# VachaLab/gorder

Hardware: AMD Instinct MI355X
Metric: trajectory frames/sec (higher is better)
Workload: dtype f32

## Files before the change

### gorder_amd/csrc/gorder_hip.hip

```cpp
#include <hip/hip_runtime.h>

#include <dlfcn.h>

#include <cmath>
#include <cstdio>
#include <cstdlib>
#include <cstring>
#include <mutex>
#include <new>
#include <string>
#include <deque>
#include <vector>

#include "../../include/gorder_hip.h"
#include "gm_math.h"
#include "plan.h"

#pragma clang fp contract(off)

using gorder::DirectItem;
using gorder::Item;
using gorder::kBlock;
using gorder::Plan;
using gorder::Tile;

#include "kernels_common.h"
#include "kernels_bonds.h"
#include "kernels_extras.h"
#include "kernels_leaflets.h"
#include "kernels_normals.h"
#include "kernels_xtc.h"


struct gorder_hip_handle {
    void *traj_cache = nullptr;
    void (*traj_cache_free)(gorder_hip_handle *) = nullptr;
    Plan plan;
    gorder_tables_t tables{};
    int device = 0;
    hipStream_t own_stream = nullptr;
    hipStream_t stream = nullptr;
    Tile *d_tiles = nullptr;
    Item *d_items = nullptr;
    uint32_t *d_tile_slots = nullptr;
    DirectItem *d_direct = nullptr;
    Tile *d_ua_tiles = nullptr;
    gorder::UaItem *d_ua_items = nullptr;
    uint32_t *d_ua_tile_slots = nullptr;
    uint32_t map_nx = 0, map_ny = 0;
    unsigned long long *d_map_sums = nullptr, *d_map_cnts = nullptr;
    unsigned long long *d_map_packed = nullptr;
    unsigned long long *d_map_rec = nullptr;
    size_t map_rec_cap = 0;
    gorder::MapRun *d_ua_runs = nullptr, *d_runs = nullptr;
    uint32_t *d_ua_run_begin = nullptr, *d_run_begin = nullptr;
    Item *d_items_by_slot = nullptr;
    uint32_t *d_ua_item_run = nullptr, *d_item_run = nullptr;
    uint4 *d_lgrid = nullptr;
    LocalRowPre *d_lrowpre = nullptr;
    LocalEdge *d_ledge = nullptr;
    float4 *d_lfinfo = nullptr;
    static constexpr uint32_t kDecidePause = 16;
    uint32_t *d_lsummary = nullptr, *h_lsummary = nullptr;
    hipEvent_t lsummary_written = nullptr;
    bool lsummary_pending = false;
    uint32_t decide_pause = 0;
    uint64_t decide_submits = 0, decide_paused_submits = 0;
    uint32_t *d_lneed = nullptr;
    uint2 *d_ltodo = nullptr;
    size_t map_lds_bytes = 0;
    bool map_staged = false;
    uint64_t map_pending = 0;
    uint64_t map_fold_limit = kMapFoldLimit;
    uint32_t map_max_mol = 1;
    unsigned long long *d_tw_sums = nullptr, *d_tw_cnts = nullptr;
    uint64_t tw_cap = 0;
    ExtraArgs extra{};
    uint32_t *d_geom_group = nullptr;
    float *d_shapes = nullptr;
    float *d_inv_box = nullptr;
    size_t inv_box_cap = 0;
    uint32_t dyn_slab = 4, local_slab = 4;
    bool local_halo = false;
    size_t local_rec_stride = 0;
    XtcCheckpoint *d_xtc_cp = nullptr;
    size_t xtc_cp_cap = 0;
    bool dyn = false;
    uint32_t *d_dyn_cloud = nullptr, *d_dyn_heads = nullptr;
    uint32_t *d_dyn_cell_of = nullptr, *d_dyn_count = nullptr;
    float *d_dyn_rec = nullptr;
// ... 407 lines not shown
        e.shapes = h->d_shapes;
        const bool ua_fast = (h->tables.flags & GORDER_FLAG_UA_FAST_NORMALISE) != 0 && !p.ua_tiles.empty();
        e.inv_box = nullptr;
        if (ua_fast && a.pbc) {
            int st3;
            if ((st3 = ensure(h, &h->d_inv_box, &h->inv_box_cap, (size_t)a.n_frames * 8)) != GORDER_OK) return st3;
            hipLaunchKernelGGL(k_inv_box, dim3((4u * a.n_frames + 255u) / 256u), dim3(256), 0, h->stream, a.box9, a.n_frames, h->d_inv_box);
            e.inv_box = h->d_inv_box;
        }
        e.dyn = (h->dyn || h->manual_active) ? h->d_dyn_normals : nullptr;
        const bool ac = (h->tables.flags & GORDER_FLAG_TRIG_ACOS_COS) != 0;
        uint32_t sub = e.maps ? (uint32_t)std::max<uint64_t>(1, (h->map_fold_limit - 1) / h->map_max_mol) : a.n_frames;
        const bool staged = e.maps && h->map_staged;
        const size_t rec_per_frame = std::max(p.ua_tiles.size() * 3u, extras ? p.tiles.size() : (size_t)0) * kBlock;
        if (staged) {
            sub = std::min<uint32_t>(sub, (uint32_t)std::max<size_t>(1, ((size_t)1 << 27) / rec_per_frame));
            sub = std::min(sub, a.n_frames);
            const int st2 = ensure(h, &h->d_map_rec, &h->map_rec_cap, rec_per_frame * (((size_t)sub + 15) / 16 * 16));
            if (st2 != GORDER_OK) return st2;
        }
        for (uint32_t lo = 0; lo < a.n_frames; lo += sub) {
            const uint32_t hi = std::min(a.n_frames, lo + sub), nf = hi - lo;
            if (e.maps) {
                const uint64_t cost = (uint64_t)nf * h->map_max_mol;
                if (h->map_pending + cost >= h->map_fold_limit) {
                    const int st = fold_maps(h);
                    if (st != GORDER_OK) return st;
                }
                h->map_pending += cost;
            }
            for (int pass = 0; pass < 2; pass++) {
                const uint32_t nt = pass == 0 ? (extras ? n_tiles : 0u) : (uint32_t)p.ua_tiles.size();
                if (!nt) continue;
                uint32_t n_chunks = std::max(1u, (h->wg_target ? h->wg_target : 8u * h->wg_capacity) / nt);
                n_chunks = std::min(n_chunks, nf);
                uint32_t fpc = (nf + n_chunks - 1) / n_chunks;
                if (staged) fpc = (fpc + 15u) / 16u * 16u;
                const bool tiled_tw = pass == 0 && e.tw && (!e.maps || staged) && !e.geom_kind && !e.dyn && !ac && !h->use_gather && h->d_item_run &&
                                      h->frames_per_stage == (int)kRecFrames && !env_flag("GORDER_HIP_TW_GATHER");
                if (tiled_tw) fpc = (fpc + kRecFrames - 1u) / kRecFrames * kRecFrames;
                n_chunks = (nf + fpc - 1) / fpc;
                FrameArgs b = a;
                b.frame0 = lo;
                b.n_frames = hi;
                b.frames_per_chunk = fpc;
                e.map_rec = staged ? h->d_map_rec : nullptr;
                e.item_run = pass == 0 ? h->d_item_run : h->d_ua_item_run;
                e.rec_frame0 = lo;
                e.rec_stride = (nf + 15u) / 16u * 16u;
                const dim3 g(pass == 0 ? nt * n_chunks : (nt * n_chunks + 7u) / 8u * 8u), blk(kBlock);
                if (pass == 0) {
                    const Item *items = (staged || tiled_tw) ? h->d_items_by_slot : h->d_items;
#define GORDER_LAUNCH_BONDS(AC, MO)                                                                               \
    hipLaunchKernelGGL((k_bonds_extras<AC, MO>), g, blk, 0, h->stream, b, e, b.xyz, b.box9, b.aflags, b.arow,       \
                       h->d_tiles, items, h->d_tile_slots, nt)
                    const bool maps_only = staged && !e.tw && !e.geom_kind && !e.dyn;
                    const bool tiled_maps = maps_only && !ac && !h->use_gather && h->frames_per_stage == (int)kRecFrames &&
                                            !env_flag("GORDER_HIP_MAPS_GATHER");
#define GORDER_LAUNCH_TM_A(NPF_, PBC_, LF_, AX_)                                                                   \
    do {                                                                                                            \
        if (tiled_tw && !staged && LF_ && h->spec_now)                                                              \
            hipLaunchKernelGGL((k_bonds_tiled_tw<NPF_, PBC_, LF_, AX_, false, LF_>), g, blk, h->lds_bytes, h->stream, b, e, b.xyz, \
                               b.box9, b.aflags, b.arow, h->d_tiles, items, h->d_tile_slots, nt, h->lw);               \
        else if (tiled_tw && staged)                                                                                \
            hipLaunchKernelGGL((k_bonds_tiled_tw<NPF_, PBC_, LF_, AX_, true>), g, blk, h->lds_bytes, h->stream, b, e, b.xyz, \
                               b.box9, b.aflags, b.arow, h->d_tiles, items, h->d_tile_slots, nt, h->lw);               \
        else if (tiled_tw)                                                                                          \
            hipLaunchKernelGGL((k_bonds_tiled_tw<NPF_, PBC_, LF_, AX_, false>), g, blk, h->lds_bytes, h->stream, b, e, b.xyz, \
                               b.box9, b.aflags, b.arow, h->d_tiles, items, h->d_tile_slots, nt, h->lw);               \
        else                                                                                                        \
            hipLaunchKernelGGL((k_bonds_tiled_maps<NPF_, PBC_, LF_, AX_>), g, blk, h->lds_bytes, h->stream, b, e, b.xyz, \
                               b.box9, b.aflags, b.arow, h->d_tiles, items, h->d_tile_slots, nt, h->lw);               \
    } while (0)
#define GORDER_LAUNCH_TM_V(NPF_, PBC_, LF_)                                                                        \
    do {                                                                                                            \
        if (h->axis == 2) GORDER_LAUNCH_TM_A(NPF_, PBC_, LF_, 2);                                                   \
        else if (h->axis == 1) GORDER_LAUNCH_TM_A(NPF_, PBC_, LF_, 1);                                              \
        else if (h->axis == 0) GORDER_LAUNCH_TM_A(NPF_, PBC_, LF_, 0);                                              \
        else GORDER_LAUNCH_TM_A(NPF_, PBC_, LF_, -1);                                                               \
    } while (0)
#define GORDER_LAUNCH_TM(NPF_)                                                                                     \
    do {                                                                                                            \
        switch ((b.pbc ? 2 : 0) | (b.leaflets ? 1 : 0)) {                                                           \
            case 0: GORDER_LAUNCH_TM_V(NPF_, false, false); break;                                                  \
            case 1: GORDER_LAUNCH_TM_V(NPF_, false, true); break;                                                   \
            case 2: GORDER_LAUNCH_TM_V(NPF_, true, false); break;                                                   \
            default: GORDER_LAUNCH_TM_V(NPF_, true, true); break;                                                   \
        }                                                                                                           \
    } while (0)
                    name(tiled_maps ? "k_bonds_tiled_maps" : (tiled_tw ? "k_bonds_tiled_tw" : "k_bonds_extras"));
                    if (tiled_maps || tiled_tw) {
                        if ((3u * p.max_window + 6u) / 4u <= 4u * 64u && !env_flag("GORDER_HIP_NPF5")) GORDER_LAUNCH_TM(4);
                        else GORDER_LAUNCH_TM(5);
                    }
                    else if (maps_only) { if (ac) GORDER_LAUNCH_BONDS(true, true); else GORDER_LAUNCH_BONDS(false, true); }
                    else { if (ac) GORDER_LAUNCH_BONDS(true, false); else GORDER_LAUNCH_BONDS(false, false); }
#undef GORDER_LAUNCH_TM
#undef GORDER_LAUNCH_TM_V
#undef GORDER_LAUNCH_TM_A
#undef GORDER_LAUNCH_BONDS
                } else {
#define GORDER_LAUNCH_UA(AC, MODE)                                                                                \
// ... 291 lines not shown
            h->map_nx = (uint32_t)fx + 1u;
            h->map_ny = (uint32_t)fy + 1u;
            const size_t nmap = 3 * (size_t)p.n_acc * h->map_nx * h->map_ny;
            HIP_TRY(h, hipMalloc((void **)&h->d_map_sums, nmap * sizeof(unsigned long long)));
            HIP_TRY(h, hipMalloc((void **)&h->d_map_cnts, nmap * sizeof(unsigned long long)));
            HIP_TRY(h, hipMemset(h->d_map_sums, 0, nmap * sizeof(unsigned long long)));
            HIP_TRY(h, hipMemset(h->d_map_cnts, 0, nmap * sizeof(unsigned long long)));
            const size_t npk = (t->leaflets.method != GORDER_LEAFLETS_NONE ? 2 : 1) * (nmap / 3);
            HIP_TRY(h, hipMalloc((void **)&h->d_map_packed, npk * sizeof(unsigned long long)));
            HIP_TRY(h, hipMemset(h->d_map_packed, 0, npk * sizeof(unsigned long long)));
            const size_t lds_bytes = npk / p.n_acc * sizeof(unsigned long long);
            h->map_lds_bytes = lds_bytes;
            if (lds_bytes <= 150u * 1024u && !env_flag("GORDER_HIP_MAP_DIRECT")) {
                if ((st = upload(h, &h->d_ua_runs, p.ua_runs)) != GORDER_OK) return st;
                if ((st = upload(h, &h->d_ua_run_begin, p.ua_run_begin)) != GORDER_OK) return st;
                if ((st = upload(h, &h->d_runs, p.runs)) != GORDER_OK) return st;
                if ((st = upload(h, &h->d_run_begin, p.run_begin)) != GORDER_OK) return st;
                if ((st = upload(h, &h->d_items_by_slot, p.items_by_slot)) != GORDER_OK) return st;
                if ((st = upload(h, &h->d_ua_item_run, p.ua_item_run)) != GORDER_OK) return st;
                HIP_TRY(h, hipFuncSetAttribute(reinterpret_cast<const void *>(k_map_accumulate),
                                               hipFuncAttributeMaxDynamicSharedMemorySize, (int)lds_bytes));
                h->map_staged = true;
            }
            e.maps = 1; e.plane = om.plane; e.x0 = om.span_x[0]; e.y0 = om.span_y[0];
            e.binx = om.bin[0]; e.biny = om.bin[1]; e.nx = h->map_nx; e.ny = h->map_ny;
            e.inv_binx = 1.0f / om.bin[0]; e.inv_biny = 1.0f / om.bin[1];
            e.bin_core = (om.bin[0] >= 0x1p-40f && om.bin[0] <= 0x1p+40f && om.bin[1] >= 0x1p-40f && om.bin[1] <= 0x1p+40f) ? 1 : 0;
            e.map_packed = h->d_map_packed;
        }
        e.tw = t->timewise ? 1 : 0;
        if (t->timewise && !p.tiles.empty()) {
            if (!h->d_items_by_slot && (st = upload(h, &h->d_items_by_slot, p.items_by_slot)) != GORDER_OK) return st;
            if ((st = upload(h, &h->d_item_run, p.item_run)) != GORDER_OK) return st;
        }
        const gorder_geometry_t &ge = t->geometry;
        if (ge.kind != GORDER_GEOM_NONE) {
            if (ge.kind > GORDER_GEOM_SPHERE || ge.reference > GORDER_GEOMREF_GROUP || ge.orientation > 2)
                return fail(h, GORDER_ERR_INVALID_ARGUMENT, "geometry kind/reference/orientation");
            if (ge.reference == GORDER_GEOMREF_BOX_CENTER && !t->handle_pbc)
                return fail(h, GORDER_ERR_INVALID_ARGUMENT, "box-centre reference needs handle_pbc (pbc.rs:243-245)");
            if (ge.reference == GORDER_GEOMREF_POINT && t->handle_pbc &&
                !(ge.structure_box[0] > 0.0f && ge.structure_box[1] > 0.0f && ge.structure_box[2] > 0.0f))
                return fail(h, GORDER_ERR_INVALID_ARGUMENT, "geometry.structure_box");
            if (ge.reference == GORDER_GEOMREF_GROUP) {
                if (!ge.group || ge.n_group == 0) return fail(h, GORDER_ERR_INVALID_ARGUMENT, "geometry.group");
                std::vector<uint32_t> grp(ge.group, ge.group + ge.n_group);
                for (uint32_t a : grp)
                    if (a >= t->n_atoms) return fail(h, GORDER_ERR_INVALID_ARGUMENT, "geometry group index out of range");
                if ((st = upload(h, &h->d_geom_group, grp)) != GORDER_OK) return st;
            }
            e.geom_kind = (int)ge.kind; e.geom_invert = ge.invert ? 1 : 0; e.geom_orient = (int)ge.orientation;
            e.geom_thr = local_radius_threshold(ge.radius);
            h->tables.geometry.group = nullptr;
        }
        if ((e.maps || e.tw || e.geom_kind) && !p.direct.empty())
            return fail(h, GORDER_ERR_INVALID_ARGUMENT,
                        "ordermaps / timewise / geometry need every bond to fit an atom window");
    }
    HIP_TRY(h, hipMalloc((void **)&h->d_err, (kErrWords + 2u) * sizeof(uint32_t)));
    HIP_TRY(h, hipMemset(h->d_err, 0xff, kErrWords * sizeof(uint32_t)));
    HIP_TRY(h, hipMemset(h->d_err + kErrWords, 0, 2u * sizeof(uint32_t)));
    h->acc_words = 4 * (size_t)p.n_acc + 1;
    HIP_TRY(h, hipMalloc((void **)&h->d_acc, h->acc_words * sizeof(unsigned long long)));
    HIP_TRY(h, hipMemset(h->d_acc, 0, h->acc_words * sizeof(unsigned long long)));
    if (const char *e = getenv("GORDER_HIP_MAP_FOLD_LIMIT")) {
        const long v = atol(e);
// ... 179 lines not shown
                HIP_TRY(h, hipMalloc((void **)&h->d_lsummary, 2 * sizeof(uint32_t)));
                HIP_TRY(h, hipMemset(h->d_lsummary, 0, 2 * sizeof(uint32_t)));
                HIP_TRY(h, hipHostMalloc((void **)&h->h_lsummary, 2 * sizeof(uint32_t)));
                h->h_lsummary[0] = h->h_lsummary[1] = 0u;
                HIP_TRY(h, hipEventCreateWithFlags(&h->lsummary_written, hipEventDisableTiming));
                HIP_TRY(h, hipFuncSetAttribute(reinterpret_cast<const void *>(k_local_decide), hipFuncAttributeMaxDynamicSharedMemorySize,
                                               (int)kDecideLds));
                HIP_TRY(h, hipFuncSetAttribute(reinterpret_cast<const void *>(k_local_sums), hipFuncAttributeMaxDynamicSharedMemorySize,
                                               (int)kSumsLds));
                HIP_TRY(h, hipMalloc((void **)&h->d_ltodo, (1 + sl * (size_t)(p.n_mol_total ? p.n_mol_total : 1)) * sizeof(uint2)));
            }
        }
        HIP_TRY(h, hipMalloc((void **)&h->d_adist, sizeof(float) * (p.n_mol_total ? p.n_mol_total : 1)));
    }
    HIP_TRY(h, hipDeviceSynchronize());
    return GORDER_OK;
}

void gorder_hip_destroy(gorder_hip_handle *h) {
    if (!h) return;
    (void)hipSetDevice(h->device);
    if (h->stream) (void)hipStreamSynchronize(h->stream);
    if (h->traj_cache_free) h->traj_cache_free(h);
    for (hipEvent_t ev : h->timing_ev)
        if (ev) (void)hipEventDestroy(ev);
    (void)hipFree(h->d_mol_slot0);
    (void)hipFree(h->d_tiles); (void)hipFree(h->d_items); (void)hipFree(h->d_tile_slots);
    (void)hipFree(h->d_direct); (void)hipFree(h->d_err); (void)hipFree(h->d_xtc_cp);
    (void)hipFree(h->d_ua_tiles); (void)hipFree(h->d_ua_items); (void)hipFree(h->d_ua_tile_slots);
    (void)hipFree(h->d_map_sums); (void)hipFree(h->d_map_cnts); (void)hipFree(h->d_map_packed); (void)hipFree(h->d_tw_sums); (void)hipFree(h->d_tw_cnts);
    (void)hipFree(h->d_geom_group); (void)hipFree(h->d_shapes); (void)hipFree(h->d_inv_box);
    (void)hipFree(h->d_map_rec); (void)hipFree(h->d_ua_runs); (void)hipFree(h->d_ua_run_begin);
    (void)hipFree(h->d_runs); (void)hipFree(h->d_run_begin); (void)hipFree(h->d_items_by_slot);
    (void)hipFree(h->d_ua_item_run); (void)hipFree(h->d_item_run); (void)hipFree(h->d_lgrid); (void)hipFree(h->d_lrowpre); (void)hipFree(h->d_ledge);
    (void)hipFree(h->d_own); (void)hipFree(h->d_mom); (void)hipFree(h->d_head_z); (void)hipFree(h->d_own_head_begin); (void)hipFree(h->d_own_heads); (void)hipFree(h->d_spec_center); (void)hipFree(h->d_spec_ok);
    (void)hipFree(h->d_spec_counters); (void)hipFree(h->d_spec_mol_begin); (void)hipFree(h->d_spec_samples);
    if (h->h_spec_counters) (void)hipHostFree(h->h_spec_counters);
    for (hipEvent_t ev : h->spec_counters_copied) if (ev) (void)hipEventDestroy(ev); (void)hipFree(h->d_lfinfo); (void)hipFree(h->d_ltodo); (void)hipFree(h->d_lneed);
    (void)hipFree(h->d_lsummary); if (h->h_lsummary) (void)hipHostFree(h->h_lsummary); if (h->lsummary_written) (void)hipEventDestroy(h->lsummary_written);
    (void)hipFree(h->d_dyn_cloud); (void)hipFree(h->d_dyn_heads); (void)hipFree(h->d_dyn_cell_of); (void)hipFree(h->d_dyn_count);
    (void)hipFree(h->d_dyn_rec); (void)hipFree(h->d_dyn_normals); (void)hipFree(h->d_dyn_cov);
    if (!h->acc_external) (void)hipFree(h->d_acc);
    (void)hipFree(h->d_rep);
    (void)hipFree(h->d_heads); (void)hipFree(h->d_membrane); (void)hipFree(h->d_methyl_begin);
    (void)hipFree(h->d_methyl_atoms); (void)hipFree(h->d_aflags); (void)hipFree(h->d_adist);
    (void)hipFree(h->d_sph_spill); (void)hipFree(h->d_sph_stats);
    (void)hipFree(h->d_arow); (void)hipFree(h->d_aframes);
    (void)hipFree(h->d_lcell_of); (void)hipFree(h->d_lcell_count); (void)hipFree(h->d_lcell_fill);
    (void)hipFree(h->d_ltrig);
    for (int k = 0; k < 2; k++) {
        (void)hipFree(h->d_stage_xyz[k]); (void)hipFree(h->d_stage_box[k]);
        if (h->stage_copied[k]) (void)hipEventDestroy(h->stage_copied[k]);
        if (h->stage_computed[k]) (void)hipEventDestroy(h->stage_computed[k]);
    }
    if (h->copy_stream) (void)hipStreamDestroy(h->copy_stream);
    if (h->own_stream) (void)hipStreamDestroy(h->own_stream);
    delete h;
}

uint32_t gorder_hip_n_accumulators(const gorder_hip_handle *h) { return h ? h->plan.n_acc : 0; }
uint32_t gorder_hip_ordermap_dims(const gorder_hip_handle *h, uint32_t *nx, uint32_t *ny) {
    if (nx) *nx = h ? h->map_nx : 0;
    if (ny) *ny = h ? h->map_ny : 0;
    return h ? h->map_nx * h->map_ny : 0;
}

int gorder_hip_set_stream(gorder_hip_handle *h, void *hip_stream) {
// ... 801 lines not shown
```

### gorder_amd/csrc/kernels_extras.h

```cpp
#pragma once

namespace {

struct ExtraArgs {
    int maps;
    uint32_t plane;
    float x0, y0, binx, biny;
    uint32_t nx, ny;
    unsigned long long *map_packed;
    unsigned long long *map_rec;
    const uint32_t *item_run;
    uint32_t rec_frame0, rec_stride;
    const float4 *dyn;
    int bin_core;
    float inv_binx, inv_biny;
    int axis;
    int tw;
    unsigned long long *tw_sums;
    unsigned long long *tw_cnts;
    unsigned long long tw_row0;
    float sin_tet, cos_tet, sin_ch3, cos_ch3, sin_half, cos_half;
    int geom_kind, geom_invert, geom_orient;
    float geom_thr;
    const float *shapes;
// ... 280 lines not shown
        if (active) S::template compute_tail<1>(a, t, it, f_full, f_end, lds, lw, acc, bad, nan_which, nan_frame, &mo);
        rec_store(e, tile_id, f_full, tid, words);
        __syncthreads();
    }
    if (nan_frame != kNoNan)
        raise_error(a.err, GORDER_ERR_UNDEFINED_POSITION, nan_frame, kStageTypes, tile_slots[t.slot0 + it.lslot], 1, it.mol, nan_which);
    if (bad) raise_box_range(a.err, f_begin);
    __syncthreads();
    unsigned long long *l_s = reinterpret_cast<unsigned long long *>(lds);
    uint32_t *l_n = reinterpret_cast<uint32_t *>(l_s + 2 * kBlock);
    l_s[tid] = 0; l_s[kBlock + tid] = 0; l_n[tid] = 0; l_n[kBlock + tid] = 0;
    __syncthreads();
    if (active && acc.n_tot) {
        atomicAdd(&l_s[it.lslot], (unsigned long long)acc.s_tot);
        atomicAdd(&l_n[it.lslot], acc.n_tot);
        if (acc.n_up) {
            atomicAdd(&l_s[kBlock + it.lslot], (unsigned long long)acc.s_up);
            atomicAdd(&l_n[kBlock + it.lslot], acc.n_up);
        }
    }
    __syncthreads();
    if (tid < t.n_slots && l_n[tid]) {
        unsigned long long *accp = a.rep + (size_t)(blockIdx.x % a.n_rep) * 4u * a.n_acc;
        const uint32_t slot = tile_slots[t.slot0 + tid];
        atomicAdd(&accp[slot], l_s[tid]);
        atomicAdd(&accp[2u * a.n_acc + slot], (unsigned long long)l_n[tid]);
        if (l_n[kBlock + tid]) {
            atomicAdd(&accp[a.n_acc + slot], l_s[kBlock + tid]);
            atomicAdd(&accp[3u * a.n_acc + slot], (unsigned long long)l_n[kBlock + tid]);
        }
    }
}

template <int NPF, bool PBC, bool LEAF, int AXIS, bool MAPS, bool MOM = false>
__global__ __launch_bounds__(kBlock, 4) void k_bonds_tiled_tw(FrameArgs a_in, ExtraArgs e, const float *__restrict__ xyz,
                                                             const float *__restrict__ box9, const uint8_t *__restrict__ aflags,
                                                             const uint32_t *__restrict__ arow, const Tile *__restrict__ tiles,
                                                             const Item *__restrict__ items, const uint32_t *__restrict__ tile_slots,
                                                             uint32_t n_tiles, uint32_t lw) {
    constexpr int G = (int)kRecFrames;
    extern __shared__ __attribute__((aligned(16))) float lds[];
    __shared__ int l_tick[kRecFrames][kBlock];
    __shared__ uint8_t l_side[kRecFrames][kBlock];
    __shared__ uint32_t l_slot_run[kBlock];
    __shared__ uint32_t l_slot_id[kBlock];
    using S = TiledStage<G, NPF, false, PBC, LEAF, AXIS>;
    FrameArgs a = a_in;
    a.xyz = xyz; a.box9 = box9; a.aflags = aflags; a.arow = arow;
    const uint32_t tile_id = blockIdx.x % n_tiles, chunk = blockIdx.x / n_tiles;
    const Tile t = tiles[tile_id];
    const uint32_t tid = threadIdx.x;
    const uint32_t sk = tid / S::TPF, si = tid % S::TPF;
    const bool active = tid < t.n_items;
    Item it{0, 0, 0, 0, 0};
    if (active) {
        it = items[t.item0 + tid];
        const uint32_t run = e.item_run[t.item0 + tid];
        if ((run >> 16) == tid) l_slot_run[it.lslot] = run;
    }
    const uint32_t f_begin = a.frame0 + chunk * a.frames_per_chunk;
    const uint32_t f_end = min(a.n_frames, f_begin + a.frames_per_chunk);
    unsigned long long words[kRecFrames], mwords[MAPS ? kRecFrames : 1];
    TiledMapOut mo{};
    if (MAPS) {
        mo.plane = e.plane; mo.x0 = e.x0; mo.y0 = e.y0; mo.binx = e.binx; mo.biny = e.biny; mo.nx = e.nx; mo.ny = e.ny;
        mo.bin_core = e.bin_core; mo.words = mwords; mo.ticks = words;
    } else {
        mo.nx = 0;
        mo.words = words;
    }
    SampleAcc acc;
    int bad = 0;
    uint32_t nan_which = 0, nan_frame = kNoNan;
    v4f pre[NPF];
    const uint32_t my_slot = tid < t.n_slots ? tile_slots[t.slot0 + tid] : 0u;
    l_slot_id[tid] = my_slot;
    uint2 own = make_uint2(0u, 0u), my_head = make_uint2(0u, 0xffffffffu);
    if (MOM) {
        own = a.own[tile_id];
        const uint32_t hq = a.own_head_begin[tile_id] + (tid & 63u);
        if (hq < a.own_head_begin[tile_id + 1u]) my_head = a.own_heads[hq];
    }
    if (f_begin + G <= f_end) S::template load<false>(a, t, f_begin, f_end, sk, si, pre);
    for (uint32_t fs = f_begin; fs < f_end; fs += G) {
        const bool full = fs + G <= f_end;
        bool finite;
        if (full) {
            finite = S::template store<false, MOM>(a, t, fs, f_end, sk, si, pre, lds, lw);
        } else {
            S::template load<true>(a, t, fs, f_end, sk, si, pre);
            finite = S::template store<true, MOM>(a, t, fs, f_end, sk, si, pre, lds, lw);
        }
        __syncthreads();
        if (full && fs + 2u * G <= f_end) S::template load<false>(a, t, fs + G, f_end, sk, si, pre);
        if (MOM && fs + sk < f_end) {
            static_assert(!MOM || (uint32_t)G * 64u == kBlock, "a wave per frame slot");
            tiled_moments(a, t, own, tile_id, n_tiles, fs + sk, lds + (size_t)sk * lw, finite, my_head);
        }
#pragma unroll
        for (uint32_t k = 0; k < kRecFrames; k++) { words[k] = kMapNoSample; if (MAPS) mwords[k] = kMapNoSample; }
        if (active) {
            if (full) S::template compute<MAPS ? 3 : 2>(a, t, it, fs, lds, lw, acc, bad, nan_which, nan_frame, &mo);
            else S::template compute_tail<MAPS ? 3 : 2>(a, t, it, fs, f_end, lds, lw, acc, bad, nan_which, nan_frame, &mo);
        }
        if constexpr (MAPS) rec_store(e, tile_id, fs, tid, mwords);
#pragma unroll
        for (uint32_t k = 0; k < kRecFrames; k++) {
            l_tick[k][tid] = (int)(uint32_t)words[k];
            l_side[k][tid] = words[k] == kMapNoSample ? (uint8_t)2 : (uint8_t)(words[k] >> 32);
        }
        __syncthreads();
        for (uint32_t w = tid; w < kRecFrames * t.n_slots; w += kBlock) {
            const uint32_t k = w % kRecFrames, ls = w / kRecFrames;
            if (fs + k >= f_end) continue;
            const uint32_t run = l_slot_run[ls], tid0 = run >> 16, n = run & 0xffffu;
            int s_all = 0, s_low = 0;
            uint32_t n_all = 0, n_low = 0;
            for (uint32_t j = 0; j < n; j++) {
                const uint32_t side = l_side[k][tid0 + j];
                const int tick = l_tick[k][tid0 + j];
                if (side == 2u) continue;
                s_all += tick; n_all += 1u;
                if (side == 1u) { s_low += tick; n_low += 1u; }
            }
            if (!n_all) continue;
            const uint32_t slot = l_slot_id[ls];
            const size_t row = ((size_t)e.tw_row0 + fs + k) * 3u * a.n_acc;
            atomicAdd(&e.tw_sums[row + slot], (unsigned long long)(long long)s_all);
            atomicAdd(&e.tw_cnts[row + slot], (unsigned long long)n_all);
            if (LEAF) {
                const uint32_t n_up = n_all - n_low;
                if (n_up) {
                    atomicAdd(&e.tw_sums[row + (size_t)a.n_acc + slot], (unsigned long long)(long long)(s_all - s_low));
                    atomicAdd(&e.tw_cnts[row + (size_t)a.n_acc + slot], (unsigned long long)n_up);
                }
            }
        }
    }
    __syncthreads();
    if (nan_frame != kNoNan)
        raise_error(a.err, GORDER_ERR_UNDEFINED_POSITION, nan_frame, kStageTypes, tile_slots[t.slot0 + it.lslot], 1, it.mol, nan_which);
    if (bad) raise_box_range(a.err, f_begin);
    unsigned long long *l_s = reinterpret_cast<unsigned long long *>(lds);
    uint32_t *l_n = reinterpret_cast<uint32_t *>(l_s + 2 * kBlock);
    l_s[tid] = 0; l_s[kBlock + tid] = 0; l_n[tid] = 0; l_n[kBlock + tid] = 0;
    __syncthreads();
    if (active && acc.n_tot) {
        atomicAdd(&l_s[it.lslot], (unsigned long long)acc.s_tot);
        atomicAdd(&l_n[it.lslot], acc.n_tot);
        if (acc.n_up) {
            atomicAdd(&l_s[kBlock + it.lslot], (unsigned long long)acc.s_up);
            atomicAdd(&l_n[kBlock + it.lslot], acc.n_up);
        }
    }
    __syncthreads();
    if (tid < t.n_slots && l_n[tid]) {
        unsigned long long *accp = a.rep + (size_t)(blockIdx.x % a.n_rep) * 4u * a.n_acc;
        atomicAdd(&accp[my_slot], l_s[tid]);
        atomicAdd(&accp[2u * a.n_acc + my_slot], (unsigned long long)l_n[tid]);
        if (l_n[kBlock + tid]) {
            atomicAdd(&accp[a.n_acc + my_slot], l_s[kBlock + tid]);
            atomicAdd(&accp[3u * a.n_acc + my_slot], (unsigned long long)l_n[kBlock + tid]);
        }
    }
}

struct V3 { float x, y, z; };
__device__ __forceinline__ V3 v3_cross(V3 a, V3 b) { return {a.y * b.z - a.z * b.y, a.z * b.x - a.x * b.z, a.x * b.y - a.y * b.x}; }
__device__ __forceinline__ float v3_norm(V3 a) { return __builtin_sqrtf((a.x * a.x + a.y * a.y) + a.z * a.z); }
__device__ __forceinline__ V3 v3_unit(V3 a) { const float n = v3_norm(a); return {a.x / n, a.y / n, a.z / n}; }
__device__ __forceinline__ V3 v3_rotate(V3 u, float s, float c, V3 v) {
    const float sqx = u.x * u.x, sqy = u.y * u.y, sqz = u.z * u.z, omc = 1.0f - c;
    const float m11 = sqx + (1.0f - sqx) * c, m12 = u.x * u.y * omc - u.z * s, m13 = u.x * u.z * omc + u.y * s;
    const float m21 = u.x * u.y * omc + u.z * s, m22 = sqy + (1.0f - sqy) * c, m23 = u.y * u.z * omc - u.x * s;
    const float m31 = u.x * u.z * omc - u.y * s, m32 = u.y * u.z * omc + u.x * s, m33 = sqz + (1.0f - sqz) * c;
    return {(m11 * v.x + m12 * v.y) + m13 * v.z, (m21 * v.x + m22 * v.y) + m23 * v.z,
            (m31 * v.x + m32 * v.y) + m33 * v.z};
}
struct PbcStep {
    V3 box;
    bool pbc;
    bool slow = false;
    int bad = 0;
    __device__ __forceinline__ float len(int k) const { return k == 0 ? box.x : (k == 1 ? box.y : box.z); }
    __device__ __forceinline__ float mi(float d, int k) { return pbc ? gm_min_image_step(d, len(k), slow) : d; }
    __device__ __forceinline__ float wr(float x, int k) {
        if (!pbc) return x;
        const float L = len(k);
        const float r = x > L ? x - L : (x < 0.0f ? x + L : x);
// ... 781 lines not shown
```

### gorder_amd/csrc/plan.h

```cpp
#pragma once
#include <algorithm>
#include <map>
#include <tuple>
#include <cstdint>
#include <utility>
#include <vector>

#include "../../include/gorder_hip.h"

namespace gorder {

#ifndef GORDER_BLOCK
#define GORDER_BLOCK 256
#endif
constexpr uint32_t kBlock = GORDER_BLOCK;
constexpr uint32_t kMaxWindow = 1024;

struct Item {
    uint16_t li, lj;
    uint16_t lslot;
    uint16_t pad;
    uint32_t mol;
};
struct Tile {
// ... 1 lines not shown
    uint32_t item0, n_items;
    uint32_t slot0, n_slots;
};
struct DirectItem {
    uint32_t i, j, slot, mol;
};
struct UaItem {
    uint16_t l[4];
    uint16_t lslot0;
    uint16_t kind;
    uint32_t mol;
};

struct MapRun {
    uint32_t tile, tid0, n, k;
};

struct Plan {
    uint32_t n_atoms = 0, n_acc = 0, n_mol_total = 0;
    uint32_t max_window = 0;
    std::vector<Tile> tiles;
    std::vector<Item> items;
    std::vector<uint32_t> tile_slots;
    std::vector<DirectItem> direct;
    std::vector<Tile> ua_tiles;
    std::vector<UaItem> ua_items;
    std::vector<uint32_t> ua_tile_slots;
    std::vector<MapRun> ua_runs;
    std::vector<uint32_t> ua_run_begin;
    std::vector<Item> items_by_slot;
    std::vector<uint32_t> item_run, ua_item_run;
    std::vector<MapRun> runs;
    std::vector<uint32_t> run_begin;
    std::vector<uint32_t> mol0;
    std::vector<uint32_t> slot0;
    bool spec_ok = false;
    std::vector<uint32_t> own;
    std::vector<uint32_t> own_head_begin;
    std::vector<uint32_t> own_heads;
};

struct Sample {
    uint32_t i, j, slot, mol;
};
struct UaSample {
    uint32_t a[4];
    uint32_t slot0, kind, mol, type;
};

inline uint32_t bank_conflict_cycles(const Item *items, uint32_t n) {
    uint32_t extra = 0;
    for (uint32_t h = 0; h < n; h += 32u)
        for (int which = 0; which < 2; which++) {
            uint16_t seen[32][8];
            uint32_t cnt[32] = {0};
            uint32_t worst = 1;
            for (uint32_t q = h; q < std::min(n, h + 32u); q++) {
                const uint16_t at = which ? items[q].lj : items[q].li;
                uint32_t &c = cnt[at % 32u];
                bool dup = false;
                for (uint32_t k = 0; k < std::min(c, 8u); k++) dup = dup || seen[at % 32u][k] == at;
                if (!dup) { if (c < 8u) seen[at % 32u][c] = at; c++; }
                worst = std::max(worst, c);
            }
            extra += worst - 1u;
        }
// ... 3 lines not shown
    constexpr uint32_t kHalf = 32;
    if (n <= kHalf) return;
    const uint32_t n_bins = (n + kHalf - 1) / kHalf;
    auto cap = [&](uint32_t b) { return b + 1 < n_bins ? kHalf : n - kHalf * (n_bins - 1); };
    struct Bin {
        std::vector<uint16_t> at_i[kHalf], at_j[kHalf];
        std::vector<Item> got;
    };
    std::vector<Bin> bins(n_bins);
    auto added = [](const std::vector<uint16_t> &v, uint16_t a) {
        return (!v.empty() && std::find(v.begin(), v.end(), a) == v.end()) ? 1u : 0u;
    };
    for (uint32_t q = 0; q < n; q++) {
        const Item it = items[q];
        uint32_t best = n_bins, best_cost = ~0u;
        size_t best_fill = 0;
        for (uint32_t b = 0; b < n_bins; b++) {
            Bin &bin = bins[b];
            if (bin.got.size() >= cap(b)) continue;
            const uint32_t cost = added(bin.at_i[it.li % kHalf], it.li) + added(bin.at_j[it.lj % kHalf], it.lj);
            if (cost < best_cost || (cost == best_cost && bin.got.size() > best_fill)) {
                best = b; best_cost = cost; best_fill = bin.got.size();
            }
        }
        Bin &bin = bins[best];
        auto note = [](std::vector<uint16_t> &v, uint16_t a) { if (std::find(v.begin(), v.end(), a) == v.end()) v.push_back(a); };
        note(bin.at_i[it.li % kHalf], it.li);
        note(bin.at_j[it.lj % kHalf], it.lj);
        bin.got.push_back(it);
    }
    std::vector<Item> order;
    for (uint32_t b = 0; b < n_bins; b++) order.insert(order.end(), bins[b].got.begin(), bins[b].got.end());
    if (5u * bank_conflict_cycles(order.data(), n) <= 4u * bank_conflict_cycles(items, n)) std::copy(order.begin(), order.end(), items);
}

inline int build_plan(const gorder_tables_t &t, bool force_direct, Plan &p, bool ua_quads = true) {
    p = Plan();
    p.n_atoms = t.n_atoms;
    if (t.n_atoms == 0 || (t.n_molecule_types && !t.molecule_types)) return GORDER_ERR_INVALID_ARGUMENT;
    std::vector<Sample> samples;
    std::vector<UaSample> ua_samples;
    uint32_t slot = 0, mol = 0;
    for (uint32_t m = 0; m < t.n_molecule_types; m++) {
        const gorder_moltype_t &mt = t.molecule_types[m];
        p.mol0.push_back(mol);
        p.slot0.push_back(slot);
        if (mt.n_bond_types && !mt.bonds) return GORDER_ERR_INVALID_ARGUMENT;
        for (uint32_t bt = 0; bt < mt.n_bond_types; bt++) {
            for (uint32_t k = 0; k < mt.n_molecules; k++) {
                const uint32_t *b = mt.bonds + 2 * ((size_t)bt * mt.n_molecules + k);
                if (b[0] >= t.n_atoms || b[1] >= t.n_atoms || b[0] == b[1]) return GORDER_ERR_INVALID_ARGUMENT;
                samples.push_back({b[0], b[1], slot + bt, mol + k});
            }
        }
        slot += mt.n_bond_types;
        if (mt.n_ua_atoms && !mt.ua_atoms) return GORDER_ERR_INVALID_ARGUMENT;
        for (uint32_t a = 0; a < mt.n_ua_atoms; a++) {
            const uint32_t kind = mt.ua_atoms[a].kind;
            if (kind < GORDER_UA_CH1_SAT || kind > GORDER_UA_CH1_UNSAT || !mt.ua_atoms[a].indices)
                return GORDER_ERR_INVALID_ARGUMENT;
            const uint32_t nidx = kind == GORDER_UA_CH1_SAT ? 4u : 3u;
            for (uint32_t k = 0; k < mt.n_molecules; k++) {
                const uint32_t *ix = mt.ua_atoms[a].indices + 4 * (size_t)k;
                UaSample us{{ix[0], ix[1], ix[2], nidx == 4 ? ix[3] : ix[1]}, slot, kind, mol + k, m};
                for (uint32_t q = 0; q < nidx; q++)
                    if (ix[q] >= t.n_atoms) return GORDER_ERR_INVALID_ARGUMENT;
// ... 223 lines not shown
                        p.items[nt[0].item0 + q].li = (uint16_t)(p.items[nt[0].item0 + q].li + shift0);
                        p.items[nt[0].item0 + q].lj = (uint16_t)(p.items[nt[0].item0 + q].lj + shift0);
                    }
                p.tiles = nt;
                p.max_window = std::max(p.max_window, widest);
                p.own = own;
                p.spec_ok = true;
            }
        }
    }
    {
        p.items_by_slot = p.items;
        std::vector<std::pair<uint32_t, MapRun>> run_of_slot;
        for (uint32_t ti = 0; ti < p.tiles.size(); ti++) {
            const Tile &tile = p.tiles[ti];
            std::stable_sort(p.items_by_slot.begin() + tile.item0, p.items_by_slot.begin() + tile.item0 + tile.n_items,
                             [](const Item &x, const Item &y) { return x.lslot < y.lslot; });
            p.item_run.resize((size_t)tile.item0 + tile.n_items, 0u);
            for (uint32_t i = 0; i < tile.n_items;) {
                const uint16_t ls = p.items_by_slot[tile.item0 + i].lslot;
                uint32_t n = 1;
                while (i + n < tile.n_items && p.items_by_slot[tile.item0 + i + n].lslot == ls) n++;
                run_of_slot.push_back({p.tile_slots[tile.slot0 + ls], MapRun{ti, i, n, 0}});
                for (uint32_t j = 0; j < n; j++) p.item_run[tile.item0 + i + j] = (i << 16) | n;
                i += n;
            }
        }
        std::stable_sort(run_of_slot.begin(), run_of_slot.end(),
                         [](const std::pair<uint32_t, MapRun> &x, const std::pair<uint32_t, MapRun> &y) { return x.first < y.first; });
        p.run_begin.assign((size_t)p.n_acc + 1, 0);
        for (const auto &r : run_of_slot) { p.run_begin[r.first + 1]++; p.runs.push_back(r.second); }
        for (uint32_t sl = 0; sl < p.n_acc; sl++) p.run_begin[sl + 1] += p.run_begin[sl];
    }
    return GORDER_OK;
}

inline int selfcheck_plan(const gorder_tables_t &t, const Plan &p) {
    std::vector<Sample> want, got;
    uint32_t slot = 0, mol = 0;
    for (uint32_t m = 0; m < t.n_molecule_types; m++) {
        const gorder_moltype_t &mt = t.molecule_types[m];
        for (uint32_t bt = 0; bt < mt.n_bond_types; bt++)
            for (uint32_t k = 0; k < mt.n_molecules; k++) {
                const uint32_t *b = mt.bonds + 2 * ((size_t)bt * mt.n_molecules + k);
                want.push_back({b[0], b[1], slot + bt, mol + k});
            }
        slot += mt.n_bond_types;
        for (uint32_t a = 0; a < mt.n_ua_atoms; a++) {
            const uint32_t kind = mt.ua_atoms[a].kind;
            slot += kind == GORDER_UA_CH3 ? 3 : kind == GORDER_UA_CH2 ? 2 : 1;
        }
        mol += mt.n_molecules;
    }
    for (const Tile &tile : p.tiles) {
        if (tile.n_items == 0 || tile.n_items > kBlock) return 1;
        if (tile.n_window == 0 || tile.n_window > kMaxWindow) return 2;
        if ((uint64_t)tile.atom0 + tile.n_window > t.n_atoms) return 3;
        if (tile.n_slots == 0 || tile.n_slots > tile.n_items) return 4;
        for (uint32_t q = 0; q < tile.n_items; q++) {
            const Item &it = p.items[tile.item0 + q];
            if (it.li >= tile.n_window || it.lj >= tile.n_window || it.lslot >= tile.n_slots) return 5;
            got.push_back({tile.atom0 + it.li, tile.atom0 + it.lj, p.tile_slots[tile.slot0 + it.lslot], it.mol});
        }
    }
    for (const DirectItem &d : p.direct) got.push_back({d.i, d.j, d.slot, d.mol});
    auto cmp = [](const Sample &a, const Sample &b) {
// ... 54 lines not shown
```

Baseline: 21.00 million.

## Fold consecutive same-layout tiles into one timewise block to cut row atomics

Tiles that share slot and run layout are grouped, up to 8 per group, and a single block walks the tiles of a group in turn for each frame group. Per-slot, per-frame sums are accumulated in extra LDS across the group and written to the timewise rows with one set of global atomics at the end, rather than once per tile. This is meant to reduce global atomic traffic and contention on the tw_sums and tw_cnts rows. In exchange it adds LDS use, which can lower occupancy, reduces the number of workgroup units, adds serial work per block, and moves NaN error reporting inside the loop.

```diff
diff --git a/gorder_amd/csrc/gorder_hip.hip b/gorder_amd/csrc/gorder_hip.hip
--- a/gorder_amd/csrc/gorder_hip.hip
+++ b/gorder_amd/csrc/gorder_hip.hip
@@ -56,6 +56,8 @@
     uint32_t *d_ua_run_begin = nullptr, *d_run_begin = nullptr;
     Item *d_items_by_slot = nullptr;
     uint32_t *d_ua_item_run = nullptr, *d_item_run = nullptr;
+    uint32_t *d_tw_groups = nullptr;
+    uint32_t n_tw_groups = 0, tw_fold_slots = 0;
     uint4 *d_lgrid = nullptr;
     LocalRowPre *d_lrowpre = nullptr;
     LocalEdge *d_ledge = nullptr;
@@ -529,12 +531,13 @@
             for (int pass = 0; pass < 2; pass++) {
                 const uint32_t nt = pass == 0 ? (extras ? n_tiles : 0u) : (uint32_t)p.ua_tiles.size();
                 if (!nt) continue;
-                uint32_t n_chunks = std::max(1u, (h->wg_target ? h->wg_target : 8u * h->wg_capacity) / nt);
+                const bool tiled_tw = pass == 0 && e.tw && (!e.maps || staged) && !e.geom_kind && !e.dyn && !ac && !h->use_gather && h->d_item_run &&
+                                      h->frames_per_stage == (int)kRecFrames && !env_flag("GORDER_HIP_TW_GATHER");
+                const uint32_t n_units = tiled_tw ? h->n_tw_groups : nt;
+                uint32_t n_chunks = std::max(1u, (h->wg_target ? h->wg_target : 8u * h->wg_capacity) / n_units);
                 n_chunks = std::min(n_chunks, nf);
                 uint32_t fpc = (nf + n_chunks - 1) / n_chunks;
                 if (staged) fpc = (fpc + 15u) / 16u * 16u;
-                const bool tiled_tw = pass == 0 && e.tw && (!e.maps || staged) && !e.geom_kind && !e.dyn && !ac && !h->use_gather && h->d_item_run &&
-                                      h->frames_per_stage == (int)kRecFrames && !env_flag("GORDER_HIP_TW_GATHER");
                 if (tiled_tw) fpc = (fpc + kRecFrames - 1u) / kRecFrames * kRecFrames;
                 n_chunks = (nf + fpc - 1) / fpc;
                 FrameArgs b = a;
@@ -545,9 +548,10 @@
                 e.item_run = pass == 0 ? h->d_item_run : h->d_ua_item_run;
                 e.rec_frame0 = lo;
                 e.rec_stride = (nf + 15u) / 16u * 16u;
-                const dim3 g(pass == 0 ? nt * n_chunks : (nt * n_chunks + 7u) / 8u * 8u), blk(kBlock);
+                const dim3 g(pass == 0 ? n_units * n_chunks : (nt * n_chunks + 7u) / 8u * 8u), blk(kBlock);
                 if (pass == 0) {
                     const Item *items = (staged || tiled_tw) ? h->d_items_by_slot : h->d_items;
+                    const size_t tw_fold_lds = (size_t)kRecFrames * h->tw_fold_slots * (b.leaflets ? 24u : 12u);
 #define GORDER_LAUNCH_BONDS(AC, MO)                                                                               \
     hipLaunchKernelGGL((k_bonds_extras<AC, MO>), g, blk, 0, h->stream, b, e, b.xyz, b.box9, b.aflags, b.arow,       \
                        h->d_tiles, items, h->d_tile_slots, nt)
@@ -557,14 +561,17 @@
 #define GORDER_LAUNCH_TM_A(NPF_, PBC_, LF_, AX_)                                                                   \
     do {                                                                                                            \
         if (tiled_tw && !staged && LF_ && h->spec_now)                                                              \
-            hipLaunchKernelGGL((k_bonds_tiled_tw<NPF_, PBC_, LF_, AX_, false, LF_>), g, blk, h->lds_bytes, h->stream, b, e, b.xyz, \
-                               b.box9, b.aflags, b.arow, h->d_tiles, items, h->d_tile_slots, nt, h->lw);               \
+            hipLaunchKernelGGL((k_bonds_tiled_tw<NPF_, PBC_, LF_, AX_, false, LF_>), g, blk, h->lds_bytes + tw_fold_lds, h->stream, b, e, b.xyz, \
+                               b.box9, b.aflags, b.arow, h->d_tiles, items, h->d_tile_slots, nt, h->lw,                \
+                               reinterpret_cast<const uint2 *>(h->d_tw_groups), h->n_tw_groups, (uint32_t)h->lds_bytes); \
         else if (tiled_tw && staged)                                                                                \
-            hipLaunchKernelGGL((k_bonds_tiled_tw<NPF_, PBC_, LF_, AX_, true>), g, blk, h->lds_bytes, h->stream, b, e, b.xyz, \
-                               b.box9, b.aflags, b.arow, h->d_tiles, items, h->d_tile_slots, nt, h->lw);               \
+            hipLaunchKernelGGL((k_bonds_tiled_tw<NPF_, PBC_, LF_, AX_, true>), g, blk, h->lds_bytes + tw_fold_lds, h->stream, b, e, b.xyz, \
+                               b.box9, b.aflags, b.arow, h->d_tiles, items, h->d_tile_slots, nt, h->lw,                \
+                               reinterpret_cast<const uint2 *>(h->d_tw_groups), h->n_tw_groups, (uint32_t)h->lds_bytes); \
         else if (tiled_tw)                                                                                          \
-            hipLaunchKernelGGL((k_bonds_tiled_tw<NPF_, PBC_, LF_, AX_, false>), g, blk, h->lds_bytes, h->stream, b, e, b.xyz, \
-                               b.box9, b.aflags, b.arow, h->d_tiles, items, h->d_tile_slots, nt, h->lw);               \
+            hipLaunchKernelGGL((k_bonds_tiled_tw<NPF_, PBC_, LF_, AX_, false>), g, blk, h->lds_bytes + tw_fold_lds, h->stream, b, e, b.xyz, \
+                               b.box9, b.aflags, b.arow, h->d_tiles, items, h->d_tile_slots, nt, h->lw,                \
+                               reinterpret_cast<const uint2 *>(h->d_tw_groups), h->n_tw_groups, (uint32_t)h->lds_bytes); \
         else                                                                                                        \
             hipLaunchKernelGGL((k_bonds_tiled_maps<NPF_, PBC_, LF_, AX_>), g, blk, h->lds_bytes, h->stream, b, e, b.xyz, \
                                b.box9, b.aflags, b.arow, h->d_tiles, items, h->d_tile_slots, nt, h->lw);               \
@@ -922,6 +929,19 @@
         if (t->timewise && !p.tiles.empty()) {
             if (!h->d_items_by_slot && (st = upload(h, &h->d_items_by_slot, p.items_by_slot)) != GORDER_OK) return st;
             if ((st = upload(h, &h->d_item_run, p.item_run)) != GORDER_OK) return st;
+            std::vector<uint32_t> groups = p.tw_groups;
+            uint32_t fold_slots = 0;
+            for (size_t g = 0; g < groups.size(); g += 2)
+                if (groups[g + 1] > 1u) fold_slots = std::max(fold_slots, p.tiles[groups[g]].n_slots);
+            const size_t stage_lds = std::max((size_t)kFramesPerStage * (((3u * p.max_window + 3u + 3u) / 4u) * 4u) * sizeof(float), (size_t)kBlock * 24);
+            if (stage_lds + kTwStaticLds + (size_t)kRecFrames * fold_slots * 24u > 64u * 1024u) {
+                groups.clear();
+                for (uint32_t ti = 0; ti < p.tiles.size(); ti++) { groups.push_back(ti); groups.push_back(1u); }
+                fold_slots = 0;
+            }
+            if ((st = upload(h, &h->d_tw_groups, groups)) != GORDER_OK) return st;
+            h->n_tw_groups = (uint32_t)(groups.size() / 2);
+            h->tw_fold_slots = fold_slots;
         }
         const gorder_geometry_t &ge = t->geometry;
         if (ge.kind != GORDER_GEOM_NONE) {
@@ -1167,7 +1187,7 @@
     (void)hipFree(h->d_geom_group); (void)hipFree(h->d_shapes); (void)hipFree(h->d_inv_box);
     (void)hipFree(h->d_map_rec); (void)hipFree(h->d_ua_runs); (void)hipFree(h->d_ua_run_begin);
     (void)hipFree(h->d_runs); (void)hipFree(h->d_run_begin); (void)hipFree(h->d_items_by_slot);
-    (void)hipFree(h->d_ua_item_run); (void)hipFree(h->d_item_run); (void)hipFree(h->d_lgrid); (void)hipFree(h->d_lrowpre); (void)hipFree(h->d_ledge);
+    (void)hipFree(h->d_ua_item_run); (void)hipFree(h->d_item_run); (void)hipFree(h->d_tw_groups); (void)hipFree(h->d_lgrid); (void)hipFree(h->d_lrowpre); (void)hipFree(h->d_ledge);
     (void)hipFree(h->d_own); (void)hipFree(h->d_mom); (void)hipFree(h->d_head_z); (void)hipFree(h->d_own_head_begin); (void)hipFree(h->d_own_heads); (void)hipFree(h->d_spec_center); (void)hipFree(h->d_spec_ok);
     (void)hipFree(h->d_spec_counters); (void)hipFree(h->d_spec_mol_begin); (void)hipFree(h->d_spec_samples);
     if (h->h_spec_counters) (void)hipHostFree(h->h_spec_counters);
diff --git a/gorder_amd/csrc/kernels_extras.h b/gorder_amd/csrc/kernels_extras.h
--- a/gorder_amd/csrc/kernels_extras.h
+++ b/gorder_amd/csrc/kernels_extras.h
@@ -336,13 +336,16 @@
     }
 }
 
+constexpr size_t kTwStaticLds = (size_t)kRecFrames * kBlock * 5u + (size_t)kBlock * 8u;
 template <int NPF, bool PBC, bool LEAF, int AXIS, bool MAPS, bool MOM = false>
 __global__ __launch_bounds__(kBlock, 4) void k_bonds_tiled_tw(FrameArgs a_in, ExtraArgs e, const float *__restrict__ xyz,
                                                              const float *__restrict__ box9, const uint8_t *__restrict__ aflags,
                                                              const uint32_t *__restrict__ arow, const Tile *__restrict__ tiles,
                                                              const Item *__restrict__ items, const uint32_t *__restrict__ tile_slots,
-                                                             uint32_t n_tiles, uint32_t lw) {
+                                                             uint32_t n_tiles, uint32_t lw, const uint2 *__restrict__ groups,
+                                                             uint32_t n_groups, uint32_t fold_off) {
     constexpr int G = (int)kRecFrames;
+    constexpr bool FOLD = GORDER_TW_FOLD_MAX > 1;
     extern __shared__ __attribute__((aligned(16))) float lds[];
     __shared__ int l_tick[kRecFrames][kBlock];
     __shared__ uint8_t l_side[kRecFrames][kBlock];
@@ -351,8 +354,11 @@
     using S = TiledStage<G, NPF, false, PBC, LEAF, AXIS>;
     FrameArgs a = a_in;
     a.xyz = xyz; a.box9 = box9; a.aflags = aflags; a.arow = arow;
-    const uint32_t tile_id = blockIdx.x % n_tiles, chunk = blockIdx.x / n_tiles;
-    const Tile t = tiles[tile_id];
+    const uint32_t chunk = blockIdx.x / n_groups;
+    const uint2 grp = groups[blockIdx.x % n_groups];
+    const uint32_t tile0 = grp.x, R = FOLD ? grp.y : 1u;
+    Tile t = tiles[tile0];
+    const uint32_t n_slots = t.n_slots, slot0 = t.slot0;
     const uint32_t tid = threadIdx.x;
     const uint32_t sk = tid / S::TPF, si = tid % S::TPF;
     const bool active = tid < t.n_items;
@@ -362,6 +368,7 @@
         const uint32_t run = e.item_run[t.item0 + tid];
         if ((run >> 16) == tid) l_slot_run[it.lslot] = run;
     }
+    const uint32_t lslot = it.lslot;
     const uint32_t f_begin = a.frame0 + chunk * a.frames_per_chunk;
     const uint32_t f_end = min(a.n_frames, f_begin + a.frames_per_chunk);
     unsigned long long words[kRecFrames], mwords[MAPS ? kRecFrames : 1];
@@ -377,17 +384,30 @@
     int bad = 0;
     uint32_t nan_which = 0, nan_frame = kNoNan;
     v4f pre[NPF];
-    const uint32_t my_slot = tid < t.n_slots ? tile_slots[t.slot0 + tid] : 0u;
+    const uint32_t my_slot = tid < n_slots ? tile_slots[slot0 + tid] : 0u;
     l_slot_id[tid] = my_slot;
-    uint2 own = make_uint2(0u, 0u), my_head = make_uint2(0u, 0xffffffffu);
-    if (MOM) {
-        own = a.own[tile_id];
-        const uint32_t hq = a.own_head_begin[tile_id] + (tid & 63u);
-        if (hq < a.own_head_begin[tile_id + 1u]) my_head = a.own_heads[hq];
-    }
+    const uint32_t n_ent = kRecFrames * n_slots;
+    long long *f_sum = reinterpret_cast<long long *>(reinterpret_cast<char *>(lds) + fold_off);
+    long long *f_sup = f_sum + n_ent;
+    uint32_t *f_cnt = reinterpret_cast<uint32_t *>(f_sum + (LEAF ? 2u : 1u) * n_ent);
+    uint32_t r = 0;
     if (f_begin + G <= f_end) S::template load<false>(a, t, f_begin, f_end, sk, si, pre);
-    for (uint32_t fs = f_begin; fs < f_end; fs += G) {
+    for (uint32_t fs = f_begin; fs < f_end;) {
+        const uint32_t tile_id = tile0 + r;
         const bool full = fs + G <= f_end;
+        const uint32_t rn = r + 1u == R ? 0u : r + 1u, fn = r + 1u == R ? fs + G : fs;
+        Tile tn = t;
+        Item itn = it;
+        if (FOLD && R > 1u) {
+            tn = tiles[tile0 + rn];
+            if (active) itn = items[tn.item0 + tid];
+        }
+        uint2 own = make_uint2(0u, 0u), my_head = make_uint2(0u, 0xffffffffu);
+        if (MOM) {
+            own = a.own[tile_id];
+            const uint32_t hq = a.own_head_begin[tile_id] + (tid & 63u);
+            if (hq < a.own_head_begin[tile_id + 1u]) my_head = a.own_heads[hq];
+        }
         bool finite;
         if (full) {
             finite = S::template store<false, MOM>(a, t, fs, f_end, sk, si, pre, lds, lw);
@@ -396,7 +416,7 @@
             finite = S::template store<true, MOM>(a, t, fs, f_end, sk, si, pre, lds, lw);
         }
         __syncthreads();
-        if (full && fs + 2u * G <= f_end) S::template load<false>(a, t, fs + G, f_end, sk, si, pre);
+        if (fn + G <= f_end) S::template load<false>(a, tn, fn, f_end, sk, si, pre);
         if (MOM && fs + sk < f_end) {
             static_assert(!MOM || (uint32_t)G * 64u == kBlock, "a wave per frame slot");
             tiled_moments(a, t, own, tile_id, n_tiles, fs + sk, lds + (size_t)sk * lw, finite, my_head);
@@ -407,6 +427,10 @@
             if (full) S::template compute<MAPS ? 3 : 2>(a, t, it, fs, lds, lw, acc, bad, nan_which, nan_frame, &mo);
             else S::template compute_tail<MAPS ? 3 : 2>(a, t, it, fs, f_end, lds, lw, acc, bad, nan_which, nan_frame, &mo);
         }
+        if (nan_frame != kNoNan) {
+            raise_error(a.err, GORDER_ERR_UNDEFINED_POSITION, nan_frame, kStageTypes, tile_slots[slot0 + lslot], 1, it.mol, nan_which);
+            nan_frame = kNoNan;
+        }
         if constexpr (MAPS) rec_store(e, tile_id, fs, tid, mwords);
 #pragma unroll
         for (uint32_t k = 0; k < kRecFrames; k++) {
@@ -414,7 +438,7 @@
             l_side[k][tid] = words[k] == kMapNoSample ? (uint8_t)2 : (uint8_t)(words[k] >> 32);
         }
         __syncthreads();
-        for (uint32_t w = tid; w < kRecFrames * t.n_slots; w += kBlock) {
+        for (uint32_t w = tid; w < n_ent; w += kBlock) {
             const uint32_t k = w % kRecFrames, ls = w / kRecFrames;
             if (fs + k >= f_end) continue;
             const uint32_t run = l_slot_run[ls], tid0 = run >> 16, n = run & 0xffffu;
@@ -427,38 +451,52 @@
                 s_all += tick; n_all += 1u;
                 if (side == 1u) { s_low += tick; n_low += 1u; }
             }
+            long long g_all = s_all, g_up = s_all - s_low;
+            uint32_t n_up = n_all - n_low;
+            if (FOLD && R > 1u) {
+                if (r != 0u) {
+                    g_all += f_sum[w]; n_all += f_cnt[w];
+                    if (LEAF) { g_up += f_sup[w]; n_up += f_cnt[n_ent + w]; }
+                }
+                if (r + 1u != R) {
+                    f_sum[w] = g_all; f_cnt[w] = n_all;
+                    if (LEAF) { f_sup[w] = g_up; f_cnt[n_ent + w] = n_up; }
+                    continue;
+                }
+            }
             if (!n_all) continue;
+#ifdef GORDER_DEBUG_NOROWATOMICS
+            if (a.n_frames != 0xffffffffu) continue;
+#endif
             const uint32_t slot = l_slot_id[ls];
             const size_t row = ((size_t)e.tw_row0 + fs + k) * 3u * a.n_acc;
-            atomicAdd(&e.tw_sums[row + slot], (unsigned long long)(long long)s_all);
+            atomicAdd(&e.tw_sums[row + slot], (unsigned long long)g_all);
             atomicAdd(&e.tw_cnts[row + slot], (unsigned long long)n_all);
             if (LEAF) {
-                const uint32_t n_up = n_all - n_low;
                 if (n_up) {
-                    atomicAdd(&e.tw_sums[row + (size_t)a.n_acc + slot], (unsigned long long)(long long)(s_all - s_low));
+                    atomicAdd(&e.tw_sums[row + (size_t)a.n_acc + slot], (unsigned long long)g_up);
                     atomicAdd(&e.tw_cnts[row + (size_t)a.n_acc + slot], (unsigned long long)n_up);
                 }
             }
         }
+        t = tn; it = itn; r = rn; fs = fn;
     }
     __syncthreads();
-    if (nan_frame != kNoNan)
-        raise_error(a.err, GORDER_ERR_UNDEFINED_POSITION, nan_frame, kStageTypes, tile_slots[t.slot0 + it.lslot], 1, it.mol, nan_which);
     if (bad) raise_box_range(a.err, f_begin);
     unsigned long long *l_s = reinterpret_cast<unsigned long long *>(lds);
     uint32_t *l_n = reinterpret_cast<uint32_t *>(l_s + 2 * kBlock);
     l_s[tid] = 0; l_s[kBlock + tid] = 0; l_n[tid] = 0; l_n[kBlock + tid] = 0;
     __syncthreads();
     if (active && acc.n_tot) {
-        atomicAdd(&l_s[it.lslot], (unsigned long long)acc.s_tot);
-        atomicAdd(&l_n[it.lslot], acc.n_tot);
+        atomicAdd(&l_s[lslot], (unsigned long long)acc.s_tot);
+        atomicAdd(&l_n[lslot], acc.n_tot);
         if (acc.n_up) {
-            atomicAdd(&l_s[kBlock + it.lslot], (unsigned long long)acc.s_up);
-            atomicAdd(&l_n[kBlock + it.lslot], acc.n_up);
+            atomicAdd(&l_s[kBlock + lslot], (unsigned long long)acc.s_up);
+            atomicAdd(&l_n[kBlock + lslot], acc.n_up);
         }
     }
     __syncthreads();
-    if (tid < t.n_slots && l_n[tid]) {
+    if (tid < n_slots && l_n[tid]) {
         unsigned long long *accp = a.rep + (size_t)(blockIdx.x % a.n_rep) * 4u * a.n_acc;
         atomicAdd(&accp[my_slot], l_s[tid]);
         atomicAdd(&accp[2u * a.n_acc + my_slot], (unsigned long long)l_n[tid]);
diff --git a/gorder_amd/csrc/plan.h b/gorder_amd/csrc/plan.h
--- a/gorder_amd/csrc/plan.h
+++ b/gorder_amd/csrc/plan.h
@@ -57,6 +57,7 @@
     std::vector<uint32_t> item_run, ua_item_run;
     std::vector<MapRun> runs;
     std::vector<uint32_t> run_begin;
+    std::vector<uint32_t> tw_groups;
     std::vector<uint32_t> mol0;
     std::vector<uint32_t> slot0;
     bool spec_ok = false;
@@ -126,6 +127,37 @@
     std::vector<Item> order;
     for (uint32_t b = 0; b < n_bins; b++) order.insert(order.end(), bins[b].got.begin(), bins[b].got.end());
     if (5u * bank_conflict_cycles(order.data(), n) <= 4u * bank_conflict_cycles(items, n)) std::copy(order.begin(), order.end(), items);
+}
+
+#ifndef GORDER_TW_FOLD_MAX
+#define GORDER_TW_FOLD_MAX 8
+#endif
+inline bool tw_same_layout(const Plan &p, uint32_t x, uint32_t y) {
+    const Tile &a = p.tiles[x], &b = p.tiles[y];
+    if (a.n_items != b.n_items || a.n_slots != b.n_slots) return false;
+    for (uint32_t s = 0; s < a.n_slots; s++)
+        if (p.tile_slots[a.slot0 + s] != p.tile_slots[b.slot0 + s]) return false;
+    for (uint32_t q = 0; q < a.n_items; q++)
+        if (p.item_run[a.item0 + q] != p.item_run[b.item0 + q] ||
+            p.items_by_slot[a.item0 + q].lslot != p.items_by_slot[b.item0 + q].lslot)
+            return false;
+    return true;
+}
+inline void build_tw_groups(Plan &p, uint32_t max_fold) {
+    p.tw_groups.clear();
+    const uint32_t nt = (uint32_t)p.tiles.size();
+    for (uint32_t t0 = 0; t0 < nt;) {
+        uint32_t n = 1;
+        while (t0 + n < nt && tw_same_layout(p, t0, t0 + n)) n++;
+        for (uint32_t done = 0; done < n;) {
+            uint32_t r = 8;
+            while (r > 1 && (r > max_fold || r > n - done)) r /= 2;
+            p.tw_groups.push_back(t0 + done);
+            p.tw_groups.push_back(r);
+            done += r;
+        }
+        t0 += n;
+    }
 }
 
 inline int build_plan(const gorder_tables_t &t, bool force_direct, Plan &p, bool ua_quads = true) {
@@ -415,6 +447,7 @@
         for (const auto &r : run_of_slot) { p.run_begin[r.first + 1]++; p.runs.push_back(r.second); }
         for (uint32_t sl = 0; sl < p.n_acc; sl++) p.run_begin[sl + 1] += p.run_begin[sl];
     }
+    build_tw_groups(p, GORDER_TW_FOLD_MAX);
     return GORDER_OK;
 }
 
```

After: 20.96 million. About the same (-0.2%).
